# tianciB/VFM-VAE

Hardware: AMD Instinct MI355X
Metric: train images/sec @256^2 f16d32 (SigLIP2-L, stage-0 strong alignment) (higher is better)
Workload: dtype bf16; 1 GPU; f16d32 SigLIP2-L stage-0 strong-alignment training iteration (D+G+sync+Adam+EMA); model=VFM-VAE f16d32 (SigLIP2-L @512 + ConvNeXt decoder + DINO ViT-S D + LPIPS-VGG16), global_batch=32, batch_per_gpu=32, seq_len=1024, resolution=256, parallelism=dp1, decoder_ops=hip, d_phase_g_forward=eager

## Files before the change

### vfm-vae_amd/csrc/gemm9.hip

```cpp
#include <type_traits>

#include "vfm_common.h"

namespace {

using namespace vfm;

typedef __bf16 bf16x8 __attribute__((ext_vector_type(8)));
typedef short s16x4 __attribute__((ext_vector_type(4)));
typedef float f32x4 __attribute__((ext_vector_type(4)));
typedef unsigned v4u32 __attribute__((ext_vector_type(4)));
typedef __attribute__((address_space(3))) s16x4 lds_s16x4;
typedef __attribute__((address_space(3))) void lds_void;

constexpr int BM = 256, BN = 256, BK = 64, THREADS = 256;
constexpr int OPB = 256 * BK * 2;
constexpr int STAGE = 2 * OPB;
constexpr int LDS9P = 2 * STAGE + 8192;

struct G9Args {
    const __hip_bfloat16* A;
    const __hip_bfloat16* B;
    void* C;
    const float* bias;
    long long lda, ldb, ldc, sA, sB, sC;
    int M, N, K;
    float alpha, beta;
    int bias_mode, act;
    long long spanA, spanB, spanC;
    int reduce, S, kchunk, KTz;
    int bs;
    void* C2;
    const __hip_bfloat16* H;
    const float* rscale;
    float* rs0;
    float* rs1;
    int T, pa, pb;
    long long psA, psB;
};

__device__ __forceinline__ int kc_off(int row, int ch) { return row * 128 + 16 * (ch ^ ((row >> 1) & 7)); }
__device__ __forceinline__ int mc_swz(int row) { return ((row & 3) << 2) | ((row >> 2) & 3); }
__device__ __forceinline__ int mc_off(int row, int ch) { return row * 256 + 16 * (ch ^ mc_swz(row)); }

__device__ __forceinline__ float gelu_tanh(float x) {
    const float u = 0.7978845608028654f * fmaf(0.044715f * x, x * x, x);
    const float e = __builtin_amdgcn_exp2f(2.8853900817779268f * u);
    return 0.5f * x * (2.f - 2.f * __builtin_amdgcn_rcpf(e + 1.f));
}

__device__ __forceinline__ uint32_t pack_bf16x2(float a, float b) {
    typedef float f2 __attribute__((ext_vector_type(2)));
    typedef __bf16 b2 __attribute__((ext_vector_type(2)));
    const f2 x = {a, b};
    return __builtin_bit_cast(uint32_t, __builtin_convertvector(x, b2));
}

__device__ __forceinline__ void dma16(__amdgpu_buffer_rsrc_t rsrc, unsigned voff, unsigned soff, unsigned m0) {
    asm volatile("s_mov_b32 m0, %3\n\ts_nop 0\n\tbuffer_load_dwordx4 %0, %1, %2 offen lds" ::"v"(voff), "s"(rsrc),
                 "s"(soff), "s"(m0)
                 : "memory");
}

__device__ __forceinline__ void dma16s(__amdgpu_buffer_rsrc_t rsrc, unsigned voff0, unsigned su, unsigned m0) {
    unsigned t;
    asm volatile("v_add_u32 %0, %1, %2\n\ts_mov_b32 m0, %4\n\ts_nop 0\n\tbuffer_load_dwordx4 %0, %3, 0 offen lds"
                 : "=&v"(t)
                 : "v"(voff0), "s"(su), "s"(rsrc), "s"(m0)
                 : "memory");
}

__device__ __forceinline__ void dma16m(__amdgpu_buffer_rsrc_t rsrc, unsigned voff0, unsigned su, unsigned mb,
                                       unsigned mo) {
    unsigned t;
    asm volatile("v_add_u32 %0, %1, %2\n\ts_add_u32 m0, %4, %5\n\ts_nop 0\n\tbuffer_load_dwordx4 %0, %3, 0 offen lds"
                 : "=&v"(t)
                 : "v"(voff0), "s"(su), "s"(rsrc), "s"(mb), "s"(mo)
                 : "memory", "scc");
}

__device__ __forceinline__ void dma4(__amdgpu_buffer_rsrc_t rsrc, unsigned voff, unsigned m0) {
    asm volatile("s_mov_b32 m0, %2\n\ts_nop 0\n\tbuffer_load_dword %0, %1, 0 offen lds" ::"v"(voff), "s"(rsrc), "s"(m0)
                 : "memory");
}

template <bool KCONT>
__device__ __forceinline__ unsigned dma_voff(long long ld, int outer0, int outer_n, int u, int tid) {
    if (KCONT) {
        const int row = 32 * u + (tid >> 3), chs = (tid & 7) ^ ((row >> 1) & 7);
        const int o = min(outer0 + row, outer_n - 1);
        return (unsigned)(((long long)o * ld + 8 * chs) * 2);
    } else {
        const int h = u >> 2, row = 16 * (u & 3) + (tid >> 4), chs = (tid & 15) ^ mc_swz(row);
        int o = outer0 + 128 * h + 8 * chs;
        if (o >= outer_n) o = 0;
        return (unsigned)(((long long)row * ld + o) * 2);
    }
}

template <bool KCONT>
__device__ __forceinline__ bf16x8 frag(const unsigned char* img, int blk, int t, int lane) {
    if (KCONT) {
        return *reinterpret_cast<const bf16x8*>(img + kc_off(16 * blk + (lane & 15), 4 * t + (lane >> 4)));
    } else {
        const unsigned char* h = img + (blk >> 3) * (OPB / 2);
        const int b = blk & 7;
        const int g = lane >> 4, q = (lane >> 2) & 3, p = lane & 3;
        const int ch = 2 * b + (p >> 1);
        const int row = 32 * t + 8 * g + q;
        const s16x4 lo = __builtin_amdgcn_ds_read_tr16_b64_v4i16((lds_s16x4*)(h + mc_off(row, ch) + 8 * (p & 1)));
        const s16x4 hi = __builtin_amdgcn_ds_read_tr16_b64_v4i16((lds_s16x4*)(h + mc_off(row + 4, ch) + 8 * (p & 1)));
        return __builtin_bit_cast(bf16x8, __builtin_shufflevector(lo, hi, 0, 1, 2, 3, 4, 5, 6, 7));
    }
}

__device__ __forceinline__ void mfma_acc(f32x4& c, const bf16x8& x, const bf16x8& y) {
    asm volatile("v_mfma_f32_16x16x32_bf16 %0, %1, %2, %0" : "+a"(c) : "v"(x), "v"(y));
}

__device__ __forceinline__ void mfma_acc0(f32x4& c, const bf16x8& x, const bf16x8& y) {
    asm volatile("v_mfma_f32_16x16x32_bf16 %0, %1, %2, 0" : "=a"(c) : "v"(x), "v"(y));
}

#define SB() __builtin_amdgcn_sched_barrier(0)
#define VMCNT(n) asm volatile("s_waitcnt vmcnt(" #n ")" ::: "memory")
template <int N>
__device__ __forceinline__ void vmcnt_const() {
    static_assert(N >= 0 && N <= 63, "vmcnt range");
    asm volatile("s_waitcnt vmcnt(%0)" ::"n"(N) : "memory");
}

#ifndef G9_P3
#define G9_P3 0
#endif
#ifndef G9_PH1
#define G9_PH1 26
#endif
#ifndef G9_PH3
#define G9_PH3 21
#endif

template <bool AK, bool BKC, bool OUTF32>
__global__ __launch_bounds__(THREADS, 1) void gemm9_kernel(G9Args a) {
    extern __shared__ __attribute__((aligned(16))) unsigned char lds[];
    const int tid = threadIdx.x, lane = tid & 63;
    const int wave = __builtin_amdgcn_readfirstlane(tid >> 6);
// ... 141 lines not shown
                }
            }
            if (OUTF32) {
                const int n0c = nw + 16 * j0 + 4 * row4;
                float* cf = reinterpret_cast<float*>(crow);
                if (mok && n0c < a.N) *reinterpret_cast<f32x4*>(cf + n0c) = v0;
                if (mok && n0c + 16 < a.N) *reinterpret_cast<f32x4*>(cf + n0c + 16) = v1;
            } else {
                const uint32_t a0 = pack_bf16x2(v0[0], v0[1]), a1 = pack_bf16x2(v0[2], v0[3]);
                const uint32_t b0 = pack_bf16x2(v1[0], v1[1]), b1 = pack_bf16x2(v1[2], v1[3]);
                const auto s0 = __builtin_amdgcn_permlane16_swap(a0, b0, false, false);
                const auto s1 = __builtin_amdgcn_permlane16_swap(a1, b1, false, false);
                const int n = nw + 16 * (j0 + (row4 & 1)) + 8 * (row4 >> 1);
                if (mok && n < a.N)
                    *reinterpret_cast<uint4*>(reinterpret_cast<__hip_bfloat16*>(crow) + n) = make_uint4(s0[0], s1[0], s0[1], s1[1]);
            }
        }
    }
}

__device__ __forceinline__ void item_tile(int item, int nwg, int total, int tiles_m, int tiles_n, int& z, int& m0,
                                          int& n0) {
    const int xcd = item & 7, q8 = total >> 3, r8 = total & 7;
    const int g = (xcd < r8 ? xcd * (q8 + 1) : r8 * (q8 + 1) + (xcd - r8) * q8) + (item >> 3);
    z = g / nwg;
    const int tile = g - z * nwg;
    constexpr int GROUP = 4;
    const int gsz = GROUP * tiles_n, grp = tile / gsz, rem = tile - grp * gsz;
    const int rows_g = min(GROUP, tiles_m - grp * GROUP);
    m0 = (grp * GROUP + rem % rows_g) * BM;
    n0 = (rem / rows_g) * BN;
}

template <int EPI>
__device__ __forceinline__ void gelu_epilogue9(const G9Args& a, const f32x4 (&acc)[8][8], const float* bsl,
                                               __amdgpu_buffer_rsrc_t rC, int z, int m0, int n0, int wm, int wn,
                                               int l15, int row4, int tiles_n) {
    auto rsrc2 = [&](const void* base, long long off, long long span) __attribute__((always_inline)) {
        const long long left = base ? span - off : 0;
        return __builtin_amdgcn_make_buffer_rsrc((void*)((const char*)base + (base ? off : 0)), 0,
                                                 (int)(left > 0 ? (left < 0x7fffffffLL ? left : 0x7fffffffLL) : 0),
                                                 0x00020000);
    };
    const int mw = m0 + 128 * wm, nw = n0 + 128 * wn;
    const bool hasS = a.rscale != nullptr;
    const long long zoff = (long long)z * a.sC * 2;
    const __amdgpu_buffer_rsrc_t rC2 = rsrc2(a.C2, zoff, a.spanC);
    const __amdgpu_buffer_rsrc_t rH = rsrc2(a.H, zoff, a.spanC);
    const long long nparts = 2LL * tiles_n;
    const long long pbase = ((long long)z * nparts + 2 * (n0 / BN) + wn) * a.M;
    const __amdgpu_buffer_rsrc_t rP0 = rsrc2(a.rs0, pbase * 4, (long long)a.M * 4 * nparts * (z + 1));
    const __amdgpu_buffer_rsrc_t rP1 = rsrc2(a.rs1, pbase * 4, (long long)a.M * 4 * nparts * (z + 1));
    uint2 hn[4][2];
    auto load_h = [&](int i, uint2 (&hv)[4][2]) __attribute__((always_inline)) {
        const unsigned ob = (unsigned)((mw + 16 * i + l15) * a.ldc + nw + 4 * row4) * 2u;
#pragma unroll
        for (int jp = 0; jp < 4; ++jp) {
            hv[jp][0] = __builtin_bit_cast(uint2, __builtin_amdgcn_raw_buffer_load_b64(rH, ob + 64u * jp, 0, 0));
            hv[jp][1] = __builtin_bit_cast(uint2, __builtin_amdgcn_raw_buffer_load_b64(rH, ob + 64u * jp + 32u, 0, 0));
        }
    };
    if (EPI == 5) load_h(0, hn);
#pragma unroll
    for (int i = 0; i < 8; ++i) {
        const int ml = 128 * wm + 16 * i + l15;
        const int m = m0 + ml;
        const bool mok = m < a.M;
        const float b1v = bsl[ml], scv = hasS ? bsl[256 + ml] : 1.f;
        uint2 hc[4][2];
        if (EPI == 5) {
#pragma unroll
            for (int jp = 0; jp < 4; ++jp) {
                hc[jp][0] = hn[jp][0];
                hc[jp][1] = hn[jp][1];
            }
            if (i < 7) load_h(i + 1, hn);
        }
        float s0 = 0.f, s1 = 0.f;
#pragma unroll
        for (int jp = 0; jp < 4; ++jp) {
            const int j0 = 2 * jp, j1 = j0 + 1;
            const int n0c = nw + 16 * j0 + 4 * row4;
            const f32x4 v0 = acc[i][j0], v1 = acc[i][j1];
            uint32_t pa[2], pb[2], qa[2], qb[2];
            if (EPI == 4) {
                float h0[4], h1[4];
#pragma unroll
                for (int r = 0; r < 4; ++r) {
                    h0[r] = __builtin_bit_cast(float, (uint32_t)__builtin_bit_cast(unsigned short, __float2bfloat16(v0[r])) << 16);
                    h1[r] = __builtin_bit_cast(float, (uint32_t)__builtin_bit_cast(unsigned short, __float2bfloat16(v1[r])) << 16);
                }
                float g0[4], g1[4];
#pragma unroll
                for (int r = 0; r < 4; ++r) {
                    const float z0 = fmaf(h0[r], scv, b1v), z1 = fmaf(h1[r], scv, b1v);
                    g0[r] = z0 * gelu_parts(z0).cdf;
                    g1[r] = z1 * gelu_parts(z1).cdf;
                }
                pa[0] = pack_bf16x2(h0[0], h0[1]); pa[1] = pack_bf16x2(h0[2], h0[3]);
                pb[0] = pack_bf16x2(h1[0], h1[1]); pb[1] = pack_bf16x2(h1[2], h1[3]);
                qa[0] = pack_bf16x2(g0[0], g0[1]); qa[1] = pack_bf16x2(g0[2], g0[3]);
                qb[0] = pack_bf16x2(g1[0], g1[1]); qb[1] = pack_bf16x2(g1[2], g1[3]);
            } else {
                float d0[4], d1[4];
                const uint32_t hw[4] = {hc[jp][0].x, hc[jp][0].y, hc[jp][1].x, hc[jp][1].y};
#pragma unroll
                for (int r = 0; r < 4; ++r) {
                    const float dg0 = __builtin_bit_cast(float, (uint32_t)__builtin_bit_cast(unsigned short, __float2bfloat16(v0[r])) << 16);
                    const float dg1 = __builtin_bit_cast(float, (uint32_t)__builtin_bit_cast(unsigned short, __float2bfloat16(v1[r])) << 16);
                    const uint32_t w0 = hw[r >> 1], w1 = hw[2 + (r >> 1)];
                    const float hv0 = __builtin_bit_cast(float, (r & 1) ? (w0 & 0xffff0000u) : (w0 << 16));
                    const float hv1 = __builtin_bit_cast(float, (r & 1) ? (w1 & 0xffff0000u) : (w1 << 16));
                    const GeluParts gp0 = gelu_parts(fmaf(hv0, scv, b1v)), gp1 = gelu_parts(fmaf(hv1, scv, b1v));
                    float dz0 = dg0 * (gp0.cdf + gp0.zpdf), dz1 = dg1 * (gp1.cdf + gp1.zpdf);
                    if (!mok || n0c + r >= a.N) dz0 = 0.f;
                    if (!mok || n0c + 16 + r >= a.N) dz1 = 0.f;
                    s0 = fmaf(dz0, hv0, s0);
                    s1 += dz0;
                    s0 = fmaf(dz1, hv1, s0);
                    s1 += dz1;
                    d0[r] = dz0 * scv;
                    d1[r] = dz1 * scv;
                }
                pa[0] = pack_bf16x2(d0[0], d0[1]); pa[1] = pack_bf16x2(d0[2], d0[3]);
                pb[0] = pack_bf16x2(d1[0], d1[1]); pb[1] = pack_bf16x2(d1[2], d1[3]);
            }
            const int n = nw + 16 * (j0 + (row4 & 1)) + 8 * (row4 >> 1);
            const unsigned o = (mok && n < a.N) ? (unsigned)(((long long)m * a.ldc + n) * 2) : 0x80000000u;
            {
                const auto x0 = __builtin_amdgcn_permlane16_swap(pa[0], pb[0], false, false);
                const auto x1 = __builtin_amdgcn_permlane16_swap(pa[1], pb[1], false, false);
                const v4u32 d = {x0[0], x1[0], x0[1], x1[1]};
                __builtin_amdgcn_raw_buffer_store_b128(d, rC, o, 0, 0);
            }
            if (EPI == 4) {
                const auto x0 = __builtin_amdgcn_permlane16_swap(qa[0], qb[0], false, false);
                const auto x1 = __builtin_amdgcn_permlane16_swap(qa[1], qb[1], false, false);
                const v4u32 d = {x0[0], x1[0], x0[1], x1[1]};
                __builtin_amdgcn_raw_buffer_store_b128(d, rC2, o, 0, 0);
            }
        }
        if (EPI == 5) {
            s0 += __shfl_xor(s0, 16);
            s1 += __shfl_xor(s1, 16);
            s0 += __shfl_xor(s0, 32);
            s1 += __shfl_xor(s1, 32);
            const unsigned po = (row4 == 0 && mok) ? (unsigned)((long long)m * 4) : 0x80000000u;
            __builtin_amdgcn_raw_buffer_store_b32(__builtin_bit_cast(unsigned, s0), rP0, po, 0, 0);
            __builtin_amdgcn_raw_buffer_store_b32(__builtin_bit_cast(unsigned, s1), rP1, po, 0, 0);
        }
        SB();
    }
}

__device__ __forceinline__ void item_k_range(const G9Args& a, int z, int KT, int& v0, int& n) {
    if (a.reduce) {
        const int V = a.KTz * a.reduce * a.T;
        v0 = z * a.kchunk;
        n = min(V, v0 + a.kchunk) - v0;
    } else if (a.bs > 1) {
        const int V = KT * a.T;
        v0 = (z % a.bs) * a.kchunk;
        n = min(V, v0 + a.kchunk) - v0;
    } else {
        v0 = 0;
        n = KT * a.T;
    }
}

template <bool AK, bool BKC, bool OUTF32, int EPI, int NP = 1>
__global__ __launch_bounds__(THREADS, 1) void gemm9p_kernel(G9Args a, int total) {
    constexpr int NP_T = NP == 3 ? 6 : NP == 2 ? 3 : 1;
    extern __shared__ __attribute__((aligned(16))) unsigned char lds[];
    const int tid = threadIdx.x, lane = tid & 63;
    const int wave = __builtin_amdgcn_readfirstlane(tid >> 6);
    const int wm = wave >> 1, wn = wave & 1;
    const int tiles_m = (a.M + BM - 1) / BM, tiles_n = (a.N + BN - 1) / BN;
    const int nwg = tiles_m * tiles_n;
    const int G = gridDim.x;
    const int KT = a.K / BK;
    const unsigned m0A = (unsigned)(size_t)(lds_void*)lds + (unsigned)wave * 1024u;
    const unsigned dkA = (unsigned)(AK ? BK * 2 : BK * a.lda * 2), dkB = (unsigned)(BKC ? BK * 2 : BK * a.ldb * 2);

    const unsigned voA0 = dma_voff<AK>(a.lda, 0, 0x7fffffff, 0, tid), voB0 = dma_voff<BKC>(a.ldb, 0, 0x7fffffff, 0, tid);
    auto ustep = [&](bool kc, long long ld, int u) __attribute__((always_inline)) {
        return (unsigned)((kc ? 32LL * u * ld : 16LL * (u & 3) * ld + 128 * (u >> 2)) * 2);
    };
    int d_item = blockIdx.x, d_kt = 0, d_k = 0;
    int d_KT = KT, d_v0 = 0, d_z = 0;
    int d_term = 0, d_kk = 0;
    long long offA = 0, offB = 0;
    long long offS = 0, offR = 0;
    auto setup_dma = [&](int item) __attribute__((always_inline)) {
        int z, m0, n0;
        item_tile(item, nwg, total, tiles_m, tiles_n, z, m0, n0);
        offA = (AK ? (long long)m0 * a.lda : (long long)m0) * 2;
        offB = (BKC ? (long long)n0 * a.ldb : (long long)n0) * 2;
        d_z = a.bs > 1 ? z / a.bs : z;
        item_k_range(a, z, KT, d_v0, d_KT);
        offS = (long long)(a.bias_mode == 1 ? n0 : m0) * 4;
        offR = ((long long)z * a.M + m0) * 4;
    };
    auto rsrc = [&](const void* base, long long off, long long span) __attribute__((always_inline)) {
        const long long left = span - off;
        return __builtin_amdgcn_make_buffer_rsrc((void*)((const char*)base + off), 0,
                                                 (int)(left > 0 ? (left < 0x7fffffffLL ? left : 0x7fffffffLL) : 0),
                                                 0x00020000);
    };
    __amdgpu_buffer_rsrc_t rA = rsrc(a.A, 0, a.spanA), rB = rsrc(a.B, 0, a.spanB), rS = rA;
    const long long spanS = EPI && a.bias ? (long long)(a.bias_mode == 1 ? a.N : a.M) * 4 : 0;
    const long long spanR = EPI >= 4 && a.rscale ? (long long)a.M * 4 * (a.reduce ? 1 : 1) : 0;
    __amdgpu_buffer_rsrc_t rR = rA;
    const unsigned sl0 = (unsigned)(size_t)(lds_void*)lds + 2 * STAGE + (unsigned)wave * 256u;
    const unsigned voS = (unsigned)tid * 4u;
    auto dma = [&](int g, int buf) __attribute__((always_inline)) {
        const unsigned mb = m0A + (unsigned)buf * STAGE;
        if (g < 8) dma16m(rA, voA0, ustep(AK, a.lda, g), mb, (unsigned)(g * 4096));
        else if (g < 16) dma16m(rB, voB0, ustep(BKC, a.ldb, g - 8), mb, (unsigned)(OPB + (g - 8) * 4096));
        else if (g == 16) dma4(rS, voS, sl0 + (unsigned)(d_k & 3) * 2048u);
        else dma4(rR, voS, sl0 + (unsigned)(d_k & 3) * 2048u + 1024u);
    };
    unsigned aLo = 0, aHi = 0, aN = 0, bLo = 0, bHi = 0, bN = 0;
    auto clamp31 = [](long long left) __attribute__((always_inline)) {
        return (unsigned)(left > 0 ? (left < 0x7fffffffLL ? left : 0x7fffffffLL) : 0);
    };
    auto mk = [](unsigned lo, unsigned hi, unsigned n) __attribute__((always_inline)) {
        return __builtin_amdgcn_make_buffer_rsrc((void*)(((unsigned long long)hi << 32) | lo), 0, (int)n, 0x00020000);
    };
    auto point = [&]() __attribute__((always_inline)) {
        const bool live = d_item < total;
        int zt = d_z, kk = NP > 1 ? d_kk + (a.bs > 1 ? d_v0 / NP_T : 0) : d_kt;
        if (a.reduce) {
            const int v = NP > 1 ? d_v0 / NP_T + d_kk : d_v0 + d_kt;
            zt = v / a.KTz;
            kk = v - zt * a.KTz;
        }
        long long pofa = 0, pofb = 0;
        if (NP > 1) {
            pofa = ((a.pa >> (2 * d_term)) & 3) * a.psA;
            pofb = ((a.pb >> (2 * d_term)) & 3) * a.psB;
        }
        const long long cA = offA + (zt * a.sA + (long long)kk * (dkA / 2) + pofa) * 2;
        const long long cB = offB + (zt * a.sB + (long long)kk * (dkB / 2) + pofb) * 2;
        const unsigned long long pA = (unsigned long long)((const char*)a.A + cA);
        const unsigned long long pB = (unsigned long long)((const char*)a.B + cB);
        aLo = __builtin_amdgcn_readfirstlane((unsigned)pA);
        aHi = __builtin_amdgcn_readfirstlane((unsigned)(pA >> 32));
// ... 10 lines not shown
        asm volatile("s_add_u32 %0, %0, %6\n\ts_addc_u32 %1, %1, 0\n\ts_sub_u32 %2, %2, %6\n\ts_cselect_b32 %2, 0, %2\n\t"
                     "s_add_u32 %3, %3, %7\n\ts_addc_u32 %4, %4, 0\n\ts_sub_u32 %5, %5, %7\n\ts_cselect_b32 %5, 0, %5"
                     : "+s"(aLo), "+s"(aHi), "+s"(aN), "+s"(bLo), "+s"(bHi), "+s"(bN)
                     : "s"(dkA), "s"(dkB)
                     : "scc");
        rA = mk(aLo, aHi, aN);
        rB = mk(bLo, bHi, bN);
    };
    auto advance = [&]() __attribute__((always_inline)) {
        if (++d_kt == d_KT) {
            d_kt = 0;
            d_term = 0;
            d_kk = 0;
            d_item += G;
            ++d_k;
            if (d_item < total) setup_dma(d_item);
            point();
        } else if (NP > 1) {
            if (++d_term == a.T) {
                d_term = 0;
                ++d_kk;
            }
            point();
        } else if (a.reduce) {
            point();
        } else {
            step();
        }
    };

    f32x4 acc[8][8];
    bf16x8 fa0[8], fb0[8], fa1[8], fb1[8];
    int flane = lane;
    auto rd = [&](int h, int r, int buf) __attribute__((always_inline)) {
        const unsigned char* base = lds + buf * STAGE;
        const bool isb = (r == 1) || r >= 9;
        const int idx = r == 0 ? 0 : r == 1 ? 0 : r <= 8 ? r - 1 : r - 8;
        if (!isb) {
            const bf16x8 v = frag<AK>(base, 8 * wm + idx, h, AK ? lane : flane);
            if (h == 0) fa0[idx] = v; else fa1[idx] = v;
        } else {
            const bf16x8 v = frag<BKC>(base + OPB, 8 * wn + idx, h, BKC ? lane : flane);
            if (h == 0) fb0[idx] = v; else fb1[idx] = v;
        }
    };
    auto mf = [&](int h, int q, bool first) __attribute__((always_inline)) {
        const int j = q >> 3, i = q & 7;
        if (first && h == 0) mfma_acc0(acc[i][j], fb0[j], fa0[i]);
        else mfma_acc(acc[i][j], h ? fb1[j] : fb0[j], h ? fa1[i] : fa0[i]);
    };

    typedef typename std::conditional<OUTF32, float, __hip_bfloat16>::type TC;
    constexpr int ES = sizeof(TC);

    setup_dma(d_item);
    point();
    constexpr int NG = EPI >= 4 ? 18 : EPI ? 17 : 16;
    constexpr int D2 = 16 - G9_P3;
    constexpr int PH2 = 128 - G9_PH1 - G9_PH3;
    constexpr int PH1 = G9_PH1, PH3 = G9_PH3;
    constexpr int SP = PH2 / D2;
    static_assert(PH1 >= 16 && PH3 >= 16 && PH1 <= 64 && PH3 <= 64 && SP >= 1, "gemm9 phase split");
#pragma unroll
    for (int g = 0; g < NG; ++g) dma(g, 0);
    advance();
#pragma unroll
    for (int g = 0; g < NG; ++g) dma(g, 1);
    advance();
    if (EPI >= 4) VMCNT(18);
    else if (EPI) VMCNT(17);
    else VMCNT(16);
    __builtin_amdgcn_s_barrier();
    SB();
#pragma unroll
    for (int r = 0; r < 16; ++r) rd(0, r, 0);
// ... 58 lines not shown
                }
            }
            __builtin_amdgcn_s_barrier();
            SB();
#pragma unroll
            for (int q = 0; q < 16; ++q) {
                mf(1, 64 - PH3 + q, false);
                SB();
                rd(0, q, cur ^ 1);
                SB();
                if (G9_P3 > 0 && (q % (16 / (G9_P3 > 0 ? G9_P3 : 1))) == 1 && q / (16 / (G9_P3 > 0 ? G9_P3 : 1)) < G9_P3) {
                    dma(D2 + q / (16 / (G9_P3 > 0 ? G9_P3 : 1)), cur);
                    SB();
                }
            }
#pragma unroll
            for (int q = 64 - PH3 + 16; q < 64; ++q) mf(1, q, false);
            SB();
            if (G9_P3 > 0) {
                advance();
                SB();
            }
            ++p;
        };
        ktile(0, std::true_type{});
        int iKT, iv0;
        {
            int z_, m0_, n0_;
            item_tile(item, nwg, total, tiles_m, tiles_n, z_, m0_, n0_);
            item_k_range(a, z_, KT, iv0, iKT);
        }
        for (int t = 1; t < iKT; ++t) ktile(t, std::false_type{});
        asm volatile("s_nop 7\n\ts_nop 7\n\ts_nop 3" ::: "memory");
        int elane = lane;
        asm volatile("" : "+v"(elane));
        const int l15 = elane & 15, row4 = elane >> 4;
        int z, m0, n0;
        item_tile(item, nwg, total, tiles_m, tiles_n, z, m0, n0);
        const int mw = m0 + 128 * wm, nw = n0 + 128 * wn;
        const __amdgpu_buffer_rsrc_t rC = rsrc(a.C, z * a.sC * ES, a.C ? a.spanC : 0);
        const unsigned zc = 0u;
        const float* bsl = reinterpret_cast<const float*>(lds + 2 * STAGE + (item_k & 3) * 2048);
        auto act = [&](float x) __attribute__((always_inline)) {
            if (EPI == 2) x = gelu_tanh(x);
            else if (EPI == 3) x = x * gelu_parts(x).cdf;
            return x;
        };
        const float fcol = a.bias_mode == 1 ? 1.f : 0.f, frow = a.bias_mode == 2 ? 1.f : 0.f;
        if (EPI >= 4) {
            gelu_epilogue9<EPI>(a, acc, bsl, rC, z, m0, n0, wm, wn, l15, row4, tiles_n);
            ++item_k;
            SB();
            continue;
        }
#pragma unroll
        for (int jp = 0; jp < 4; ++jp) {
            const int j0 = 2 * jp, j1 = j0 + 1;
            const int c0 = 128 * wn + 16 * j0 + 4 * row4;
            f32x4 bc0 = {}, bc1 = {};
            if (EPI) {
                bc0 = *reinterpret_cast<const f32x4*>(bsl + c0) * fcol;
                bc1 = *reinterpret_cast<const f32x4*>(bsl + c0 + 16) * fcol;
            }
#pragma unroll
            for (int i = 0; i < 8; ++i) {
                const int m = mw + 16 * i + l15;
                const bool mok = m < a.M;
                f32x4 v0 = acc[i][j0], v1 = acc[i][j1];
                if (EPI) {
                    const float br = bsl[128 * wm + 16 * i + l15] * frow;
#pragma unroll
                    for (int r = 0; r < 4; ++r) {
                        v0[r] = act(fmaf(a.alpha, v0[r], bc0[r] + br));
                        v1[r] = act(fmaf(a.alpha, v1[r], bc1[r] + br));
                    }
                }
                if (OUTF32) {
                    const int n0c = nw + 16 * j0 + 4 * row4;
                    const unsigned o0 = (mok && n0c < a.N) ? (unsigned)(((long long)m * a.ldc + n0c) * ES) : 0x80000000u;
                    const unsigned o1 = (mok && n0c + 16 < a.N) ? (unsigned)(((long long)m * a.ldc + n0c + 16) * ES) : 0x80000000u;
                    __builtin_amdgcn_raw_buffer_store_b128(__builtin_bit_cast(v4u32, v0), rC, o0, zc, 0);
                    __builtin_amdgcn_raw_buffer_store_b128(__builtin_bit_cast(v4u32, v1), rC, o1, zc, 0);
                } else {
                    const uint32_t a0 = pack_bf16x2(v0[0], v0[1]), a1 = pack_bf16x2(v0[2], v0[3]);
                    const uint32_t b0 = pack_bf16x2(v1[0], v1[1]), b1 = pack_bf16x2(v1[2], v1[3]);
                    const auto s0 = __builtin_amdgcn_permlane16_swap(a0, b0, false, false);
                    const auto s1 = __builtin_amdgcn_permlane16_swap(a1, b1, false, false);
                    const int n = nw + 16 * (j0 + (row4 & 1)) + 8 * (row4 >> 1);
                    const unsigned o = (mok && n < a.N) ? (unsigned)(((long long)m * a.ldc + n) * ES) : 0x80000000u;
                    const v4u32 d = {s0[0], s1[0], s0[1], s1[1]};
                    __builtin_amdgcn_raw_buffer_store_b128(d, rC, o, zc, 0);
                }
                SB();
            }
        }
        ++item_k;
        SB();
    }
    VMCNT(0);
}

template <bool OUTF32>
__global__ __launch_bounds__(256) void gemm9_reduce(const float* __restrict__ ws, void* C, int M, int N, long long ldc,
                                                    int S, float alpha) {
    const long long MN = (long long)M * N;
    for (long long i4 = ((long long)blockIdx.x * 256 + threadIdx.x) * 4; i4 < MN; i4 += (long long)gridDim.x * 1024) {
        f32x4 v = *reinterpret_cast<const f32x4*>(ws + i4);
        for (int k = 1; k < S; ++k) v += *reinterpret_cast<const f32x4*>(ws + k * MN + i4);
        v *= alpha;
        const int m = (int)(i4 / N), n = (int)(i4 - (long long)m * N);
        if (OUTF32) {
            *reinterpret_cast<f32x4*>(reinterpret_cast<float*>(C) + m * ldc + n) = v;
        } else {
            const uint2 b = make_uint2(pack_bf16x2(v[0], v[1]), pack_bf16x2(v[2], v[3]));
            *reinterpret_cast<uint2*>(reinterpret_cast<__hip_bfloat16*>(C) + m * ldc + n) = b;
        }
    }
}

__global__ __launch_bounds__(256) void gemm9_reduce_batched(const float* __restrict__ ws, float* C, int M, int N,
                                                            long long ldc, long long sC, int S, float alpha) {
    const long long MN = (long long)M * N;
    const int z = blockIdx.y;
    const float* w = ws + (long long)z * S * MN;
    for (long long i4 = ((long long)blockIdx.x * 256 + threadIdx.x) * 4; i4 < MN; i4 += (long long)gridDim.x * 1024) {
        f32x4 v = *reinterpret_cast<const f32x4*>(w + i4);
        for (int k = 1; k < S; ++k) v += *reinterpret_cast<const f32x4*>(w + k * MN + i4);
        v *= alpha;
        const int m = (int)(i4 / N), n = (int)(i4 - (long long)m * N);
        *reinterpret_cast<f32x4*>(C + z * sC + m * ldc + n) = v;
    }
}

int g_persistent = 1;


template <bool AK, bool BKC>
void launch9_pieces(const G9Args& a, int batch, hipStream_t st) {
    static bool attr[MAXDEV] = {};
    const int dv_attr = cur_dev();
    if (!attr[dv_attr]) {
        (void)hipFuncSetAttribute((const void*)gemm9p_kernel<AK, BKC, true, 0, 3>, hipFuncAttributeMaxDynamicSharedMemorySize, LDS9P);
        (void)hipFuncSetAttribute((const void*)gemm9p_kernel<AK, BKC, true, 1, 3>, hipFuncAttributeMaxDynamicSharedMemorySize, LDS9P);
        attr[dv_attr] = true;
    }
    const int cus = device_cus(cur_dev());
    const int nwg = ((a.M + BM - 1) / BM) * ((a.N + BN - 1) / BN);
    const long long total = (long long)nwg * batch;
    const int grid = (int)std::min<long long>(total, cus);
    const bool plain = a.bias_mode == 0 && a.alpha == 1.f;
    if (plain)
        VFM_LAUNCH((gemm9p_kernel<AK, BKC, true, 0, 3>), dim3(grid), dim3(THREADS), LDS9P, st, a, (int)total);
    else
        VFM_LAUNCH((gemm9p_kernel<AK, BKC, true, 1, 3>), dim3(grid), dim3(THREADS), LDS9P, st, a, (int)total);
}

template <bool AK, bool BKC, bool OUTF32>
void launch9(const G9Args& a, int batch, hipStream_t st) {
    static bool attr[MAXDEV] = {};
    const int dv_attr = cur_dev();
    if (!attr[dv_attr]) {
        (void)hipFuncSetAttribute((const void*)gemm9_kernel<AK, BKC, OUTF32>, hipFuncAttributeMaxDynamicSharedMemorySize,
                                  2 * STAGE);
        attr[dv_attr] = true;
    }
    const int nwg = ((a.M + BM - 1) / BM) * ((a.N + BN - 1) / BN);
    const bool plain = a.beta == 0.f && a.bias_mode == 0 && a.act == 0 && a.alpha == 1.f;
    if (g_persistent && a.beta == 0.f) {
        static bool attrp[MAXDEV] = {};
        const int dv_attrp = cur_dev();
        if (!attrp[dv_attrp]) {
            (void)hipFuncSetAttribute((const void*)gemm9p_kernel<AK, BKC, OUTF32, 0>, hipFuncAttributeMaxDynamicSharedMemorySize, LDS9P);
            (void)hipFuncSetAttribute((const void*)gemm9p_kernel<AK, BKC, OUTF32, 1>, hipFuncAttributeMaxDynamicSharedMemorySize, LDS9P);
            (void)hipFuncSetAttribute((const void*)gemm9p_kernel<AK, BKC, OUTF32, 2>, hipFuncAttributeMaxDynamicSharedMemorySize, LDS9P);
            (void)hipFuncSetAttribute((const void*)gemm9p_kernel<AK, BKC, OUTF32, 3>, hipFuncAttributeMaxDynamicSharedMemorySize, LDS9P);
            attrp[dv_attrp] = true;
        }
        const int cus = device_cus(cur_dev());
        const long long total = (long long)nwg * (a.reduce ? a.S : batch);
        const int grid = (int)std::min<long long>(total, cus);
        if (plain)
            VFM_LAUNCH((gemm9p_kernel<AK, BKC, OUTF32, 0>), dim3(grid), dim3(THREADS), LDS9P, st, a, (int)total);
        else if (a.act == 0)
            VFM_LAUNCH((gemm9p_kernel<AK, BKC, OUTF32, 1>), dim3(grid), dim3(THREADS), LDS9P, st, a, (int)total);
        else if (a.act == 1)
            VFM_LAUNCH((gemm9p_kernel<AK, BKC, OUTF32, 2>), dim3(grid), dim3(THREADS), LDS9P, st, a, (int)total);
        else
            VFM_LAUNCH((gemm9p_kernel<AK, BKC, OUTF32, 3>), dim3(grid), dim3(THREADS), LDS9P, st, a, (int)total);
        return;
    }
    VFM_LAUNCH((gemm9_kernel<AK, BKC, OUTF32>), dim3(nwg, batch), dim3(THREADS), 2 * STAGE, st, a);
}

long long span9(int kcont, long long outer, long long kdim, long long ld, long long sb, int batch) {
    const long long rows = kcont ? outer : kdim;
    const long long cols = kcont ? kdim : outer;
    const long long e = (rows - 1) * ld + cols + (long long)(batch - 1) * sb;
    return e * 2;
}

}

static int gemm9_impl(const void* A, const void* B, void* C, const float* bias, int out_dtype, int M, int N, int K,
                      int batch, int a_kcont, long long lda, long long sA, int b_kcont, long long ldb, long long sB,
                      long long ldc, long long sC, float alpha, float beta, int bias_mode, int act, float* workspace,
                      int splits, int reduce_batch, void* stream) {
    if (!A || !B || !C || M <= 0 || N <= 0 || K <= 0 || batch <= 0 || batch > 65535) return VFM_ERR_ARGS;
    if (out_dtype != VFM_BF16 && out_dtype != VFM_F32) return VFM_NO_KERNEL;
    if (bias_mode < 0 || bias_mode > 2 || (bias_mode && !bias) || act < 0 || act > 2) return VFM_ERR_ARGS;
    if (K % BK || N % 8) return VFM_NO_KERNEL;
    const int a_c = a_kcont ? K : M, b_c = b_kcont ? K : N;
    if (a_c % 8 || b_c % 8 || lda % 8 || ldb % 8 || sA % 8 || sB % 8 || ldc % 8 || sC % 8) return VFM_NO_KERNEL;
    if (((uintptr_t)A | (uintptr_t)B | (uintptr_t)C) % 16) return VFM_NO_KERNEL;
// ... 76 lines not shown
        const int S0 = std::max(1, std::min(splits, KTz));
        const int kc = (KTz + S0 - 1) / S0;
        return (long long)M * N * batch * ((KTz + kc - 1) / kc);
    }
    const int V = (K / BK) * (reduce_batch ? batch : 1);
    const int S0 = std::max(1, std::min(splits, V));
    const int kc = (V + S0 - 1) / S0;
    const int S = (V + kc - 1) / kc;
    return (long long)M * N * S;
}

extern "C" int vfm_gemm9_gelu(const void* W, const void* X, void* C, void* C2, const void* H, const float* rscale,
                              const float* bias, float* rsum0, float* rsum1, int mode, int M, int N, int K, int batch,
                              long long lda, long long ldb, long long sB, long long ldc, long long sC, void* stream) {
    if (!W || !X || M <= 0 || N <= 0 || K <= 0 || batch <= 0 || batch > 65535) return VFM_ERR_ARGS;
    if (mode == 1 ? !C2 : (mode == 2 ? (!C || !H || !rsum1) : true)) return VFM_ERR_ARGS;
    if (K % BK || K % 8 || N % 8 || M % 8 || lda % 8 || ldb % 8 || sB % 8 || ldc % 8 || sC % 8) return VFM_NO_KERNEL;
    if (((uintptr_t)W | (uintptr_t)X | (uintptr_t)C | (uintptr_t)C2 | (uintptr_t)H) % 16) return VFM_NO_KERNEL;
    if (lda < K || ldb < N || ldc < N) return VFM_ERR_ARGS;
    if (span9(1, M, K, lda, 0, 1) >= (1LL << 31) || span9(0, N, K, ldb, 0, 1) >= (1LL << 31) ||
        ((long long)(M - 1) * ldc + N) * 2 >= (1LL << 31))
        return VFM_NO_KERNEL;
    const long long nwg = (long long)((M + BM - 1) / BM) * ((N + BN - 1) / BN);
    if (nwg * batch > 0x7fffffffLL) return VFM_ERR_ARGS;
    G9Args a{};
    a.T = 1;
    a.A = (const __hip_bfloat16*)W; a.B = (const __hip_bfloat16*)X; a.C = C; a.C2 = C2;
    a.H = (const __hip_bfloat16*)H; a.rscale = rscale; a.bias = bias; a.rs0 = rsum0; a.rs1 = rsum1;
    a.lda = lda; a.ldb = ldb; a.ldc = ldc; a.sA = 0; a.sB = sB; a.sC = sC;
    a.M = M; a.N = N; a.K = K; a.alpha = 1.f; a.beta = 0.f; a.bias_mode = 0; a.act = 0;
    a.spanA = span9(1, M, K, lda, 0, 1);
    a.spanB = span9(0, N, K, ldb, sB, batch);
    a.spanC = ((long long)(M - 1) * ldc + N + (long long)(batch - 1) * sC) * 2;
    hipStream_t st = (hipStream_t)stream;
    static bool attr[MAXDEV] = {};
    const int dv_attr = cur_dev();
    if (!attr[dv_attr]) {
        (void)hipFuncSetAttribute((const void*)gemm9p_kernel<true, false, false, 4>, hipFuncAttributeMaxDynamicSharedMemorySize, LDS9P);
        (void)hipFuncSetAttribute((const void*)gemm9p_kernel<true, false, false, 5>, hipFuncAttributeMaxDynamicSharedMemorySize, LDS9P);
        attr[dv_attr] = true;
    }
    const int cus = device_cus(cur_dev());
    const long long total = nwg * batch;
    const int grid = (int)std::min<long long>(total, cus);
    if (mode == 1)
        VFM_LAUNCH((gemm9p_kernel<true, false, false, 4>), dim3(grid), dim3(THREADS), LDS9P, st, a, (int)total);
    else
        VFM_LAUNCH((gemm9p_kernel<true, false, false, 5>), dim3(grid), dim3(THREADS), LDS9P, st, a, (int)total);
    return launch_status();
}

extern "C" int vfm_gemm9_pieces(const void* A, const void* B, float* C, const float* bias, int M, int N, int K,
                                int batch, int a_kcont, long long lda, long long sA, long long psA, int b_kcont,
                                long long ldb, long long sB, long long psB, long long ldc, long long sC, float alpha,
                                int bias_mode, float* workspace, int splits, int reduce_batch, void* stream) {
    if (!A || !B || !C || M <= 0 || N <= 0 || K <= 0 || batch <= 0 || batch > 65535) return VFM_ERR_ARGS;
    if (bias_mode < 0 || bias_mode > 2 || (bias_mode && !bias) || psA < 0 || psB < 0) return VFM_ERR_ARGS;
    if (K % BK || N % 8) return VFM_NO_KERNEL;
    const int a_c = a_kcont ? K : M, b_c = b_kcont ? K : N;
    if (a_c % 8 || b_c % 8 || lda % 8 || ldb % 8 || sA % 8 || sB % 8 || ldc % 8 || sC % 8 || psA % 8 || psB % 8)
        return VFM_NO_KERNEL;
    if (((uintptr_t)A | (uintptr_t)B | (uintptr_t)C) % 16) return VFM_NO_KERNEL;
    const int kra = (a_kcont && !psA) ? 3 * K : K, krb = (b_kcont && !psB) ? 3 * K : K;
    if (lda < (a_kcont ? (long long)kra : M) || ldb < (b_kcont ? (long long)krb : N) || ldc < N) return VFM_ERR_ARGS;
    const long long nwg = (long long)((M + BM - 1) / BM) * ((N + BN - 1) / BN);
    if (nwg * batch > 0x7fffffffLL || !g_persistent) return VFM_NO_KERNEL;
// ... 37 lines not shown
            p.C = workspace; p.ldc = N; p.sC = MN; p.alpha = 1.f;
            p.spanC = MN * (long long)batch * a.bs * 4;
            p.bias = nullptr; p.bias_mode = 0;
            go(p, batch * a.bs);
            const int blocks = (int)std::min<long long>((MN / 4 + 255) / 256, 1024);
            VFM_LAUNCH(gemm9_reduce_batched, dim3(blocks, batch), dim3(256), 0, st, workspace, C, M, N, ldc, sC, a.bs,
                       alpha);
            return launch_status();
        }
        const int KTz = K / BK, V = KTz * batch;
        const int S0 = std::max(1, std::min(splits, V));
        const int kcr = (V + S0 - 1) / S0;
        a.reduce = batch;
        a.KTz = KTz;
        a.kchunk = kcr * a.T;
        a.S = (V + kcr - 1) / kcr;
        const long long MN = (long long)M * N;
        if (MN * 4 >= (1LL << 31) || MN % 4) return VFM_NO_KERNEL;
        G9Args p = a;
        p.C = workspace; p.ldc = N; p.sC = MN; p.alpha = 1.f;
        p.spanC = MN * a.S * 4;
        p.bias = nullptr; p.bias_mode = 0;
        go(p, a.S);
        const int blocks = (int)std::min<long long>((MN / 4 + 255) / 256, 4096);
        VFM_LAUNCH(gemm9_reduce<true>, dim3(blocks), dim3(256), 0, st, workspace, C, M, N, ldc, a.S, alpha);
        return launch_status();
    }
    go(a, batch);
    return launch_status();
}

extern "C" int vfm_gemm9_gelu_parts(int N) { return N <= 0 ? -1 : 2 * ((N + BN - 1) / BN); }

extern "C" int vfm_gemm9_set_mode(int persistent) {
    const int prev = g_persistent;
    g_persistent = persistent ? 1 : 0;
    return prev;
}
```

Before: 100.1 images/sec.

## Stage GEMM epilogue stores through per-wave LDS for row-contiguous coalesced writes

Adds a per-wave LDS staging buffer so the bf16 epilogue (plain, bias/act, and fused GELU variants) transposes each 16-row slice in LDS. Each lane then issues full-row 128-bit stores, one slice behind the compute, instead of scattered column-chunk stores. This targets inefficient global write coalescing for short-K GEMMs where the epilogue is exposed. It also simplifies the K-contiguous single-partition fragment reads to precomputed lane offsets and moves lane-id computation into inline asm. A dev-only null-output switch and a benchmark script are added to measure how much epilogue cost is exposed. The extra LDS per block and LDS round-trips add cost and may reduce occupancy headroom.

```diff
diff --git a/tools_dev/g9epibench.py b/tools_dev/g9epibench.py
--- /dev/null
+++ b/tools_dev/g9epibench.py
@@ -0,0 +1,104 @@
+import argparse
+import ctypes
+import os
+import statistics
+import sys
+
+ROOT = os.path.dirname(os.path.dirname(os.path.abspath(__file__)))
+sys.path[:0] = [os.path.join(ROOT, "vfm-vae_amd"), ROOT]
+import torch
+
+from torch_utils import custom_ops
+from torch_utils.ops import decoder_hip, gemm_hip
+
+DEV = "cuda"
+BATCH = 32
+
+
+def timed(fn, iters):
+    for _ in range(3):
+        fn()
+    torch.cuda.synchronize()
+    s, e = torch.cuda.Event(enable_timing=True), torch.cuda.Event(enable_timing=True)
+    s.record()
+    for _ in range(iters):
+        fn()
+    e.record()
+    torch.cuda.synchronize()
+    return s.elapsed_time(e) / iters * 1e3
+
+
+def bf(*shape, scale=1.0):
+    return (torch.randn(*shape, device=DEV) * scale).to(torch.bfloat16)
+
+
+def shapes():
+    def plain(name, M, K, P, a_t):
+        def build():
+            W = bf(K, M, scale=K ** -0.5).t() if a_t else bf(M, K, scale=K ** -0.5)
+            x = bf(BATCH, K, P)
+            out = torch.empty(BATCH, M, P, dtype=torch.bfloat16, device=DEV)
+            return lambda: gemm_hip.try_gemm(W, x, out=out, route=("g9", 0))
+        return name, 2.0 * BATCH * M * K * P, 2.0 * BATCH * M * P, build
+
+    def gelu(name, C, P):
+        def build():
+            W1, m = bf(4 * C, C, scale=C ** -0.5), bf(BATCH, C, P)
+            s, b1 = torch.rand(BATCH, 4 * C, device=DEV) + 0.5, torch.randn(4 * C, device=DEV)
+            return lambda: decoder_hip.gemm_gelu_fwd(W1, m, s, b1, want_h=True)
+        return name, 2.0 * BATCH * 4 * C * C * P, 2.0 * 2 * BATCH * 4 * C * P, build
+
+    def tower(name, M, N, K):
+        def build():
+            A, W, b = bf(M, K), bf(N, K, scale=K ** -0.5), torch.randn(N, device=DEV)
+            out = torch.empty(M, N, dtype=torch.bfloat16, device=DEV)
+            return lambda: gemm_hip.try_gemm(A, W.t(), out=out, bias=b, bias_dim=1, act="gelu_tanh", route=("g9", 0))
+        return name, 2.0 * M * N * K, 2.0 * M * N, build
+
+    return [plain("dg b4  [1024,256]x[32,256,16384]", 1024, 256, 16384, True),
+            plain("dg b3  [2048,512]x[32,512,4096]", 2048, 512, 4096, True),
+            plain("dm b4  [256,1024]x[32,1024,16384]", 256, 1024, 16384, True),
+            gelu("pw1+gelu b4 [1024,256]x[32,256,16384]", 256, 16384),
+            gelu("pw1+gelu b3 [2048,512]x[32,512,4096]", 512, 4096),
+            plain("pw2 b4 [256,1024]x[32,1024,16384]", 256, 1024, 16384, False),
+            tower("tower fc1 32768x4096x1024 bias+tanh", 32768, 4096, 1024)]
+
+
+def main():
+    ap = argparse.ArgumentParser()
+    ap.add_argument("--iters", type=int, default=20)
+    ap.add_argument("--reps", type=int, default=3)
+    ap.add_argument("--only", default="")
+    ap.add_argument("--no-null", action="store_true", help="T_full only (a library without the dev entry point)")
+    args = ap.parse_args()
+    lib = custom_ops.get_native()
+    null_out = None
+    if not args.no_null:
+        null_out = lib.vfm_gemm9_dev_null_out
+        null_out.argtypes, null_out.restype = [ctypes.c_int], ctypes.c_int
+    print(f"# {torch.cuda.get_device_name(0)}; batch {BATCH}; {args.iters} launches per figure, {args.reps} figures "
+          f"per mode, alternating; us per launch: min (median)")
+    print(f"{'shape':42s} {'T_full':>16s} {'T_null':>16s} {'exposed':>9s} {'write@T_full':>13s} {'TF/s':>7s}")
+    for name, flops, obytes, build in shapes():
+        if args.only not in name:
+            continue
+        fn = build()
+        full, null = [], []
+        for _ in range(args.reps):
+            full.append(timed(fn, args.iters))
+            if null_out is not None:
+                null_out(1)
+                try:
+                    null.append(timed(fn, args.iters))
+                finally:
+                    null_out(0)
+        tf, tn = min(full), (min(null) if null else float("nan"))
+        print(f"{name:42s} {tf:8.1f} ({statistics.median(full):7.1f}) {tn:8.1f} "
+              f"({statistics.median(null) if null else float('nan'):7.1f}) {tf - tn:9.1f} "
+              f"{obytes / tf / 1e6:10.2f} TB/s {flops / tf / 1e6:7.1f}", flush=True)
+        del fn
+        torch.cuda.empty_cache()
+
+
+if __name__ == "__main__":
+    main()
diff --git a/vfm-vae_amd/csrc/gemm9.hip b/vfm-vae_amd/csrc/gemm9.hip
--- a/vfm-vae_amd/csrc/gemm9.hip
+++ b/vfm-vae_amd/csrc/gemm9.hip
@@ -16,7 +16,9 @@
 constexpr int BM = 256, BN = 256, BK = 64, THREADS = 256;
 constexpr int OPB = 256 * BK * 2;
 constexpr int STAGE = 2 * OPB;
-constexpr int LDS9P = 2 * STAGE + 8192;
+constexpr int SLOTS9 = 8192;
+constexpr int STG_ROW = 272, STG_WAVE = 16 * STG_ROW;
+constexpr int LDS9P = 2 * STAGE + SLOTS9 + 4 * STG_WAVE;
 
 struct G9Args {
     const __hip_bfloat16* A;
@@ -79,8 +81,12 @@
                  : "memory", "scc");
 }
 
-__device__ __forceinline__ void dma4(__amdgpu_buffer_rsrc_t rsrc, unsigned voff, unsigned m0) {
-    asm volatile("s_mov_b32 m0, %2\n\ts_nop 0\n\tbuffer_load_dword %0, %1, 0 offen lds" ::"v"(voff), "s"(rsrc), "s"(m0)
+__device__ __forceinline__ void dma4(__amdgpu_buffer_rsrc_t rsrc, unsigned woff, unsigned m0) {
+    unsigned t;
+    asm volatile("v_mbcnt_lo_u32_b32 %0, -1, 0\n\tv_mbcnt_hi_u32_b32 %0, -1, %0\n\tv_lshl_add_u32 %0, %0, 2, %2\n\t"
+                 "s_mov_b32 m0, %3\n\ts_nop 0\n\tbuffer_load_dword %0, %1, 0 offen lds"
+                 : "=&v"(t)
+                 : "s"(rsrc), "s"(woff), "s"(m0)
                  : "memory");
 }
 
@@ -112,6 +118,10 @@
         const s16x4 hi = __builtin_amdgcn_ds_read_tr16_b64_v4i16((lds_s16x4*)(h + mc_off(row + 4, ch) + 8 * (p & 1)));
         return __builtin_bit_cast(bf16x8, __builtin_shufflevector(lo, hi, 0, 1, 2, 3, 4, 5, 6, 7));
     }
+}
+
+__device__ __forceinline__ bf16x8 frag_kc1(const unsigned char* img, int blk, unsigned lp) {
+    return *reinterpret_cast<const bf16x8*>(img + blk * 2048 + lp);
 }
 
 __device__ __forceinline__ void mfma_acc(f32x4& c, const bf16x8& x, const bf16x8& y) {
@@ -319,10 +329,35 @@
     n0 = (rem / rows_g) * BN;
 }
 
-template <int EPI>
+__device__ __forceinline__ void stage_put(unsigned char* stg, int l15, int row4, int jp, const v4u32& d) {
+    *reinterpret_cast<v4u32*>(stg + l15 * STG_ROW + 16 * (4 * jp + 2 * (row4 & 1) + (row4 >> 1))) = d;
+}
+
+__device__ __forceinline__ void stage_get(const unsigned char* stg, int lane, v4u32 (&d)[4]) {
+    asm volatile("" ::: "memory");
+#pragma unroll
+    for (int k = 0; k < 4; ++k)
+        d[k] = *reinterpret_cast<const v4u32*>(stg + (4 * k + (lane >> 4)) * STG_ROW + 16 * (lane & 15));
+    asm volatile("" ::: "memory");
+}
+
+__device__ __forceinline__ void stage_send(const v4u32 (&d)[4], int lane, __amdgpu_buffer_rsrc_t rC, int mrow0, int ncol,
+                                           int M, int N, long long ldc) {
+#pragma unroll
+    for (int k = 0; k < 4; ++k) {
+        const int m = mrow0 + 4 * k + (lane >> 4);
+        const unsigned o = (m < M && ncol < N) ? (unsigned)(((long long)m * ldc + ncol) * 2) : 0x80000000u;
+        __builtin_amdgcn_raw_buffer_store_b128(d[k], rC, o, 0, 0);
+    }
+}
+
+template <int EPI, bool STG>
 __device__ __forceinline__ void gelu_epilogue9(const G9Args& a, const f32x4 (&acc)[8][8], const float* bsl,
                                                __amdgpu_buffer_rsrc_t rC, int z, int m0, int n0, int wm, int wn,
-                                               int l15, int row4, int tiles_n) {
+                                               int lane, unsigned char* stg, int tiles_n) {
+    const int l15 = lane & 15, row4 = lane >> 4;
+    constexpr bool staged = STG;
+    const int nst = n0 + 128 * wn + 8 * l15;
     auto rsrc2 = [&](const void* base, long long off, long long span) __attribute__((always_inline)) {
         const long long left = base ? span - off : 0;
         return __builtin_amdgcn_make_buffer_rsrc((void*)((const char*)base + (base ? off : 0)), 0,
@@ -348,6 +383,7 @@
         }
     };
     if (EPI == 5) load_h(0, hn);
+    v4u32 sh[4], sg[4];
 #pragma unroll
     for (int i = 0; i < 8; ++i) {
         const int ml = 128 * wm + 16 * i + l15;
@@ -364,6 +400,7 @@
             if (i < 7) load_h(i + 1, hn);
         }
         float s0 = 0.f, s1 = 0.f;
+        v4u32 gq[4];
 #pragma unroll
         for (int jp = 0; jp < 4; ++jp) {
             const int j0 = 2 * jp, j1 = j0 + 1;
@@ -418,13 +455,26 @@
                 const auto x0 = __builtin_amdgcn_permlane16_swap(pa[0], pb[0], false, false);
                 const auto x1 = __builtin_amdgcn_permlane16_swap(pa[1], pb[1], false, false);
                 const v4u32 d = {x0[0], x1[0], x0[1], x1[1]};
-                __builtin_amdgcn_raw_buffer_store_b128(d, rC, o, 0, 0);
+                if (staged) stage_put(stg, l15, row4, jp, d);
+                else __builtin_amdgcn_raw_buffer_store_b128(d, rC, o, 0, 0);
             }
             if (EPI == 4) {
                 const auto x0 = __builtin_amdgcn_permlane16_swap(qa[0], qb[0], false, false);
                 const auto x1 = __builtin_amdgcn_permlane16_swap(qa[1], qb[1], false, false);
-                const v4u32 d = {x0[0], x1[0], x0[1], x1[1]};
-                __builtin_amdgcn_raw_buffer_store_b128(d, rC2, o, 0, 0);
+                gq[jp] = v4u32{x0[0], x1[0], x0[1], x1[1]};
+                if (!staged) __builtin_amdgcn_raw_buffer_store_b128(gq[jp], rC2, o, 0, 0);
+            }
+        }
+        if (staged) {
+            if (i > 0) {
+                stage_send(sh, lane, rC, mw + 16 * (i - 1), nst, a.M, a.N, a.ldc);
+                if (EPI == 4) stage_send(sg, lane, rC2, mw + 16 * (i - 1), nst, a.M, a.N, a.ldc);
+            }
+            stage_get(stg, lane, sh);
+            if (EPI == 4) {
+#pragma unroll
+                for (int jp = 0; jp < 4; ++jp) stage_put(stg, l15, row4, jp, gq[jp]);
+                stage_get(stg, lane, sg);
             }
         }
         if (EPI == 5) {
@@ -437,6 +487,10 @@
             __builtin_amdgcn_raw_buffer_store_b32(__builtin_bit_cast(unsigned, s1), rP1, po, 0, 0);
         }
         SB();
+    }
+    if (staged) {
+        stage_send(sh, lane, rC, mw + 16 * 7, nst, a.M, a.N, a.ldc);
+        if (EPI == 4) stage_send(sg, lane, rC2, mw + 16 * 7, nst, a.M, a.N, a.ldc);
     }
 }
 
@@ -499,7 +553,7 @@
     const long long spanR = EPI >= 4 && a.rscale ? (long long)a.M * 4 * (a.reduce ? 1 : 1) : 0;
     __amdgpu_buffer_rsrc_t rR = rA;
     const unsigned sl0 = (unsigned)(size_t)(lds_void*)lds + 2 * STAGE + (unsigned)wave * 256u;
-    const unsigned voS = (unsigned)tid * 4u;
+    const unsigned voS = (unsigned)wave * 256u;
     auto dma = [&](int g, int buf) __attribute__((always_inline)) {
         const unsigned mb = m0A + (unsigned)buf * STAGE;
         if (g < 8) dma16m(rA, voA0, ustep(AK, a.lda, g), mb, (unsigned)(g * 4096));
@@ -576,15 +630,18 @@
     f32x4 acc[8][8];
     bf16x8 fa0[8], fb0[8], fa1[8], fb1[8];
     int flane = lane;
+    const unsigned lp0 = (unsigned)kc_off(lane & 15, lane >> 4), lp1 = lp0 ^ 64u;
     auto rd = [&](int h, int r, int buf) __attribute__((always_inline)) {
         const unsigned char* base = lds + buf * STAGE;
         const bool isb = (r == 1) || r >= 9;
         const int idx = r == 0 ? 0 : r == 1 ? 0 : r <= 8 ? r - 1 : r - 8;
+        constexpr bool ONE = !OUTF32 && NP == 1;
         if (!isb) {
-            const bf16x8 v = frag<AK>(base, 8 * wm + idx, h, AK ? lane : flane);
+            const bf16x8 v = AK && ONE ? frag_kc1(base, 8 * wm + idx, h ? lp1 : lp0) : frag<AK>(base, 8 * wm + idx, h, AK ? lane : flane);
             if (h == 0) fa0[idx] = v; else fa1[idx] = v;
         } else {
-            const bf16x8 v = frag<BKC>(base + OPB, 8 * wn + idx, h, BKC ? lane : flane);
+            const bf16x8 v = BKC && ONE ? frag_kc1(base + OPB, 8 * wn + idx, h ? lp1 : lp0)
+                                        : frag<BKC>(base + OPB, 8 * wn + idx, h, BKC ? lane : flane);
             if (h == 0) fb0[idx] = v; else fb1[idx] = v;
         }
     };
@@ -709,8 +766,8 @@
         }
         for (int t = 1; t < iKT; ++t) ktile(t, std::false_type{});
         asm volatile("s_nop 7\n\ts_nop 7\n\ts_nop 3" ::: "memory");
-        int elane = lane;
-        asm volatile("" : "+v"(elane));
+        int elane;
+        asm volatile("v_mbcnt_lo_u32_b32 %0, -1, 0\n\tv_mbcnt_hi_u32_b32 %0, -1, %0" : "=v"(elane));
         const int l15 = elane & 15, row4 = elane >> 4;
         int z, m0, n0;
         item_tile(item, nwg, total, tiles_m, tiles_n, z, m0, n0);
@@ -718,58 +775,100 @@
         const __amdgpu_buffer_rsrc_t rC = rsrc(a.C, z * a.sC * ES, a.C ? a.spanC : 0);
         const unsigned zc = 0u;
         const float* bsl = reinterpret_cast<const float*>(lds + 2 * STAGE + (item_k & 3) * 2048);
+        unsigned char* stg = lds + 2 * STAGE + SLOTS9 + wave * STG_WAVE;
         auto act = [&](float x) __attribute__((always_inline)) {
             if (EPI == 2) x = gelu_tanh(x);
             else if (EPI == 3) x = x * gelu_parts(x).cdf;
             return x;
         };
         const float fcol = a.bias_mode == 1 ? 1.f : 0.f, frow = a.bias_mode == 2 ? 1.f : 0.f;
+        const bool staged = !OUTF32 && (EPI == 5 || iKT <= (EPI == 4 ? 4 : 8));
         if (EPI >= 4) {
-            gelu_epilogue9<EPI>(a, acc, bsl, rC, z, m0, n0, wm, wn, l15, row4, tiles_n);
+            if (EPI == 5 || staged) gelu_epilogue9<EPI, true>(a, acc, bsl, rC, z, m0, n0, wm, wn, elane, stg, tiles_n);
+            else gelu_epilogue9<EPI, false>(a, acc, bsl, rC, z, m0, n0, wm, wn, elane, stg, tiles_n);
             ++item_k;
             SB();
             continue;
         }
-#pragma unroll
-        for (int jp = 0; jp < 4; ++jp) {
-            const int j0 = 2 * jp, j1 = j0 + 1;
-            const int c0 = 128 * wn + 16 * j0 + 4 * row4;
-            f32x4 bc0 = {}, bc1 = {};
+        if (OUTF32 || !staged) {
+#pragma unroll
+            for (int jp = 0; jp < 4; ++jp) {
+                const int j0 = 2 * jp, j1 = j0 + 1;
+                const int c0 = 128 * wn + 16 * j0 + 4 * row4;
+                f32x4 bc0 = {}, bc1 = {};
+                if (EPI) {
+                    bc0 = *reinterpret_cast<const f32x4*>(bsl + c0) * fcol;
+                    bc1 = *reinterpret_cast<const f32x4*>(bsl + c0 + 16) * fcol;
+                }
+#pragma unroll
+                for (int i = 0; i < 8; ++i) {
+                    const int m = mw + 16 * i + l15;
+                    const bool mok = m < a.M;
+                    f32x4 v0 = acc[i][j0], v1 = acc[i][j1];
+                    if (EPI) {
+                        const float br = bsl[128 * wm + 16 * i + l15] * frow;
+#pragma unroll
+                        for (int r = 0; r < 4; ++r) {
+                            v0[r] = act(fmaf(a.alpha, v0[r], bc0[r] + br));
+                            v1[r] = act(fmaf(a.alpha, v1[r], bc1[r] + br));
+                        }
+                    }
+                    if (OUTF32) {
+                        const int n0c = nw + 16 * j0 + 4 * row4;
+                        const unsigned o0 = (mok && n0c < a.N) ? (unsigned)(((long long)m * a.ldc + n0c) * ES) : 0x80000000u;
+                        const unsigned o1 = (mok && n0c + 16 < a.N) ? (unsigned)(((long long)m * a.ldc + n0c + 16) * ES) : 0x80000000u;
+                        __builtin_amdgcn_raw_buffer_store_b128(__builtin_bit_cast(v4u32, v0), rC, o0, zc, 0);
+                        __builtin_amdgcn_raw_buffer_store_b128(__builtin_bit_cast(v4u32, v1), rC, o1, zc, 0);
+                    } else {
+                        const uint32_t a0 = pack_bf16x2(v0[0], v0[1]), a1 = pack_bf16x2(v0[2], v0[3]);
+                        const uint32_t b0 = pack_bf16x2(v1[0], v1[1]), b1 = pack_bf16x2(v1[2], v1[3]);
+                        const auto s0 = __builtin_amdgcn_permlane16_swap(a0, b0, false, false);
+                        const auto s1 = __builtin_amdgcn_permlane16_swap(a1, b1, false, false);
+                        const int n = nw + 16 * (j0 + (row4 & 1)) + 8 * (row4 >> 1);
+                        const unsigned o = (mok && n < a.N) ? (unsigned)(((long long)m * a.ldc + n) * ES) : 0x80000000u;
+                        const v4u32 d = {s0[0], s1[0], s0[1], s1[1]};
+                        __builtin_amdgcn_raw_buffer_store_b128(d, rC, o, zc, 0);
+                    }
+                    SB();
+                }
+            }
+        } else {
+            f32x4 bc[4][2] = {};
             if (EPI) {
-                bc0 = *reinterpret_cast<const f32x4*>(bsl + c0) * fcol;
-                bc1 = *reinterpret_cast<const f32x4*>(bsl + c0 + 16) * fcol;
-            }
+#pragma unroll
+                for (int jp = 0; jp < 4; ++jp) {
+                    const int c0 = 128 * wn + 32 * jp + 4 * row4;
+                    bc[jp][0] = *reinterpret_cast<const f32x4*>(bsl + c0) * fcol;
+                    bc[jp][1] = *reinterpret_cast<const f32x4*>(bsl + c0 + 16) * fcol;
+                }
+            }
+            const int nst = nw + 8 * l15;
+            v4u32 sd[4];
 #pragma unroll
             for (int i = 0; i < 8; ++i) {
-                const int m = mw + 16 * i + l15;
-                const bool mok = m < a.M;
-                f32x4 v0 = acc[i][j0], v1 = acc[i][j1];
-                if (EPI) {
-                    const float br = bsl[128 * wm + 16 * i + l15] * frow;
-#pragma unroll
-                    for (int r = 0; r < 4; ++r) {
-                        v0[r] = act(fmaf(a.alpha, v0[r], bc0[r] + br));
-                        v1[r] = act(fmaf(a.alpha, v1[r], bc1[r] + br));
+                float br = 0.f;
+                if (EPI) br = bsl[128 * wm + 16 * i + l15] * frow;
+#pragma unroll
+                for (int jp = 0; jp < 4; ++jp) {
+                    f32x4 v0 = acc[i][2 * jp], v1 = acc[i][2 * jp + 1];
+                    if (EPI) {
+#pragma unroll
+                        for (int r = 0; r < 4; ++r) {
+                            v0[r] = act(fmaf(a.alpha, v0[r], bc[jp][0][r] + br));
+                            v1[r] = act(fmaf(a.alpha, v1[r], bc[jp][1][r] + br));
+                        }
                     }
-                }
-                if (OUTF32) {
-                    const int n0c = nw + 16 * j0 + 4 * row4;
-                    const unsigned o0 = (mok && n0c < a.N) ? (unsigned)(((long long)m * a.ldc + n0c) * ES) : 0x80000000u;
-                    const unsigned o1 = (mok && n0c + 16 < a.N) ? (unsigned)(((long long)m * a.ldc + n0c + 16) * ES) : 0x80000000u;
-                    __builtin_amdgcn_raw_buffer_store_b128(__builtin_bit_cast(v4u32, v0), rC, o0, zc, 0);
-                    __builtin_amdgcn_raw_buffer_store_b128(__builtin_bit_cast(v4u32, v1), rC, o1, zc, 0);
-                } else {
                     const uint32_t a0 = pack_bf16x2(v0[0], v0[1]), a1 = pack_bf16x2(v0[2], v0[3]);
                     const uint32_t b0 = pack_bf16x2(v1[0], v1[1]), b1 = pack_bf16x2(v1[2], v1[3]);
                     const auto s0 = __builtin_amdgcn_permlane16_swap(a0, b0, false, false);
                     const auto s1 = __builtin_amdgcn_permlane16_swap(a1, b1, false, false);
-                    const int n = nw + 16 * (j0 + (row4 & 1)) + 8 * (row4 >> 1);
-                    const unsigned o = (mok && n < a.N) ? (unsigned)(((long long)m * a.ldc + n) * ES) : 0x80000000u;
-                    const v4u32 d = {s0[0], s1[0], s0[1], s1[1]};
-                    __builtin_amdgcn_raw_buffer_store_b128(d, rC, o, zc, 0);
+                    stage_put(stg, l15, row4, jp, v4u32{s0[0], s1[0], s0[1], s1[1]});
                 }
+                if (i > 0) stage_send(sd, elane, rC, mw + 16 * (i - 1), nst, a.M, a.N, a.ldc);
+                stage_get(stg, elane, sd);
                 SB();
             }
+            stage_send(sd, elane, rC, mw + 16 * 7, nst, a.M, a.N, a.ldc);
         }
         ++item_k;
         SB();
@@ -810,6 +909,7 @@
 }
 
 int g_persistent = 1;
+int g_null_out = 0;
 
 
 template <bool AK, bool BKC>
@@ -856,6 +956,9 @@
         const int cus = device_cus(cur_dev());
         const long long total = (long long)nwg * (a.reduce ? a.S : batch);
         const int grid = (int)std::min<long long>(total, cus);
+        G9Args an = a;
+        if (g_null_out && !a.reduce) an.C = nullptr;
+        const G9Args& a = an;
         if (plain)
             VFM_LAUNCH((gemm9p_kernel<AK, BKC, OUTF32, 0>), dim3(grid), dim3(THREADS), LDS9P, st, a, (int)total);
         else if (a.act == 0)
@@ -998,6 +1101,7 @@
     a.spanA = span9(1, M, K, lda, 0, 1);
     a.spanB = span9(0, N, K, ldb, sB, batch);
     a.spanC = ((long long)(M - 1) * ldc + N + (long long)(batch - 1) * sC) * 2;
+    if (g_null_out && mode == 1) a.C = a.C2 = nullptr;
     hipStream_t st = (hipStream_t)stream;
     static bool attr[MAXDEV] = {};
     const int dv_attr = cur_dev();
@@ -1101,6 +1205,12 @@
 
 extern "C" int vfm_gemm9_gelu_parts(int N) { return N <= 0 ? -1 : 2 * ((N + BN - 1) / BN); }
 
+extern "C" int vfm_gemm9_dev_null_out(int on) {
+    const int prev = g_null_out;
+    g_null_out = on ? 1 : 0;
+    return prev;
+}
+
 extern "C" int vfm_gemm9_set_mode(int persistent) {
     const int prev = g_persistent;
     g_persistent = persistent ? 1 : 0;
```

Measured after the change: 100.8 images/sec (median of 6 runs). Within noise of the previous version (+0.6%).
